# JuliaSmoothOptimizers/CaNNOLeS.jl

Hardware: AMD Instinct MI355X
Metric: Newton systems/sec (fp64), batched n=1e4 NLS; achieved HBM GB/s vs peak (higher is better)
Workload: dtype f64; 1 GPU; cfg3 band constrained NLS n=10000 nequ=10000 ncon=50, 16384 independent problems per GPU, one newton_system! per problem per step; batch_per_gpu=16384, total_problems=16384, ordering=canonical+early, nnzL_stored=145150, nnzL_exact=100180, fronts=1000, all_success=True

## Files before the change

### cannoles.jl_amd/csrc/band.hip

```cpp
#include <hip/hip_runtime.h>

#include "band.h"
#include "kernels.h"

namespace cnl {

namespace {

template <class T>
__device__ __forceinline__ T* as_global(T* p) {
  return (T*)(__attribute__((address_space(1))) T*)p;
}

typedef const __attribute__((address_space(4))) int* cptr;
__device__ __forceinline__ cptr as_const(const int* p) { return (cptr)(const __attribute__((address_space(1))) int*)p; }

constexpr int NPC = BAND_NPIECE;
constexpr int LANE_D = BAND_LANE_DOUBLES;
constexpr int EXCH_OFF = BAND_IN_OFF;
static_assert(48 <= BAND_NPIECE * 8, "exchange area inside the operand pieces");

__device__ __forceinline__ constexpr int sidx(int a, int b) { return a >= b ? a * (a + 1) / 2 + b : b * (b + 1) / 2 + a; }

template <class T>
__device__ __forceinline__ T rrcp(T d) {
  T r;
  if constexpr (sizeof(T) == 8) r = __builtin_amdgcn_rcp(d);
  else r = __builtin_amdgcn_rcpf(d);
  const T e = fma(-d, r, T(1));
  return fma(r, e, r);
}
template <class T>
__device__ __forceinline__ T rdiv(T w, T d, T r) {
  const T q = w * r;
  const T res = fma(-d, q, w);
  return fma(res, r, q);
}


constexpr int NS = BAND_NS;
template <class T>
struct Win {
  T S[NS * (NS + 1) / 2];
  T X[NS];
  T S55;
  T c[NS];
  T c5;
};
__device__ __forceinline__ constexpr int lslot(int PH, int k) { return (PH - BAND_HW + k + NS) % NS; }

#define LDSD(off) (*reinterpret_cast<const T*>(myb + (off)))
#define LDSW(off) (*reinterpret_cast<T*>(myb + (off)))

struct Rec { int v[BAND_SW]; };
struct RowRec { int v[BAND_RW]; };
__device__ __forceinline__ void load_rec(Rec& R, const char* recb, int o) {
  const int4* q = reinterpret_cast<const int4*>(recb + 4 * o);
#pragma unroll
  for (int k = 0; k < BAND_SW / 4; k++) { const int4 t = q[k]; R.v[4 * k] = t.x; R.v[4 * k + 1] = t.y; R.v[4 * k + 2] = t.z; R.v[4 * k + 3] = t.w; }
}
__device__ __forceinline__ void load_row(RowRec& R, const char* recb, int o) {
  const int4* q = reinterpret_cast<const int4*>(recb + 4 * o);
#pragma unroll
  for (int k = 0; k < BAND_RW / 4; k++) { const int4 t = q[k]; R.v[4 * k] = t.x; R.v[4 * k + 1] = t.y; R.v[4 * k + 2] = t.z; R.v[4 * k + 3] = t.w; }
}

template <class T>
struct FOps { T eo[15]; T rj[BAND_NB]; T rdr, rrr; };
template <class T>
__device__ __forceinline__ void fload(FOps<T>& P, const Rec& st, const RowRec& row0, const int fl, char* myb) {
#pragma unroll
  for (int q = 0; q < 15; q++) P.eo[q] = LDSD(st.v[BS_DG0 + q]);
  static_assert(BS_RX == BS_DG0 + 14, "the fifteen operands of an entering variable are consecutive words of the step block");
  P.rdr = T(1); P.rrr = T(0);
#pragma unroll
  for (int k = 0; k < BAND_NB; k++) P.rj[k] = T(0);
  if ((fl >> 8) & 255) {
#pragma unroll
    for (int k = 0; k < BAND_NB; k++) P.rj[k] = LDSD(row0.v[BR_J0 + k]);
    P.rdr = LDSD(row0.v[BR_DI]);
    P.rrr = LDSD(row0.v[BR_RR]);
  }
}

__device__ __forceinline__ long long band_il_offset(int e, int stride) { return stride ? (long long)(e >> 3) * stride + (e & 7) : (long long)e; }

template <int PH, class T>
__device__ __forceinline__ void fstep(Win<T>& W, const FOps<T>& OP, const Rec& st, const int fl, const char* recb, const int o, char* myb,
                                      const T* __restrict__ gvals, const T* __restrict__ grhs, cptr borders, long long pv, long long pr,
                                      bool has_rhs, T rho, bool ovr, T tol, int& npos, int& nzer, const int vstride = 0, const int rstride = 0) {
  constexpr int es = PH, ps = lslot(PH, 0);
  const int nrows = (fl >> 8) & 255;
  const T (&eo)[15] = OP.eo;
  const T (&rj)[BAND_NB] = OP.rj;
  const T rdr = OP.rdr, rrr = OP.rrr;
  {
    const T dg = (eo[0] + eo[1]) + eo[2];
    T rv = eo[BS_RHO - BS_DG0];
    if (!(fl & (1 << 16))) rv = ovr ? rho : rv;
    W.S[sidx(es, es)] = dg + rv;
#pragma unroll
    for (int k = 1; k <= BAND_HW; k++) W.S[sidx(es, lslot(PH, BAND_HW - k))] = eo[BS_OD - BS_DG0 + 2 * (k - 1)] + eo[BS_OD - BS_DG0 + 2 * (k - 1) + 1];
    W.X[es] = eo[BS_BC0 - BS_DG0] + eo[BS_BC1 - BS_DG0];
    W.c[es] = eo[BS_RX - BS_DG0];
  }
  for (int i = 0; i < nrows; i++) {
    T J[BAND_NB], dr, rr;
    if (i == 0) {
#pragma unroll
      for (int k = 0; k < BAND_NB; k++) J[k] = rj[k];
      dr = rdr; rr = rrr;
    } else {
      RowRec rb;
      load_row(rb, recb, o + BAND_SW + BAND_RW * i);
#pragma unroll
      for (int k = 0; k < BAND_NB; k++) J[k] = LDSD(rb.v[BR_J0 + k]);
      dr = LDSD(rb.v[BR_DI]);
      rr = LDSD(rb.v[BR_RR]);
    }
    npos += dr > tol;
    nzer += fabs(dr) <= tol;
    const T r = rrcp(dr);
    const T w = rdiv(T(-1), dr, r);
    const T tr = rr * w;
#pragma unroll
    for (int ka = 0; ka < BAND_NB; ka++) {
      const T ta = J[ka] * w;
#pragma unroll
      for (int kb = 0; kb <= ka; kb++) W.S[sidx(lslot(PH, ka), lslot(PH, kb))] = fma(ta, J[kb], W.S[sidx(lslot(PH, ka), lslot(PH, kb))]);
      W.c[lslot(PH, ka)] = fma(tr, J[ka], W.c[lslot(PH, ka)]);
    }
  }
  if (fl & BF_PIVOT_B) {
    cptr bt = borders + BAND_BW * __builtin_amdgcn_readfirstlane(st.v[BS_BORDER]);
    W.S55 += gvals[pv + band_il_offset(bt[BB_DSRC], vstride)];
    W.c5 += has_rhs ? grhs[pr + band_il_offset(bt[BB_RHS], rstride)] : T(0);
    const T d = W.S55;
    npos += d > tol;
    nzer += fabs(d) <= tol;
    const T r = rrcp(d);
    T l[BAND_NB], w[BAND_NB];
#pragma unroll
    for (int k = 0; k < BAND_NB; k++) { w[k] = W.X[lslot(PH, k)]; l[k] = rdiv(w[k], d, r); }
    const T z = rdiv(W.c5, d, r);
#pragma unroll
    for (int ka = 0; ka < BAND_NB; ka++) {
#pragma unroll
      for (int kb = 0; kb <= ka; kb++) W.S[sidx(lslot(PH, ka), lslot(PH, kb))] = fma(w[ka], -l[kb], W.S[sidx(lslot(PH, ka), lslot(PH, kb))]);
      W.c[lslot(PH, ka)] = fma(w[ka], -z, W.c[lslot(PH, ka)]);
    }
    T* lo = reinterpret_cast<T*>(myb + st.v[BS_LB]);
#pragma unroll
    for (int k = 0; k < BAND_NB; k++) lo[k] = l[k];
    lo[BAND_NB] = z;
#pragma unroll
    for (int k = 0; k < BAND_NB; k++) W.X[lslot(PH, k)] = T(0);
    W.S55 = T(0); W.c5 = T(0);
  }
  if (fl & BF_PIVOT_X) {
    const T d = W.S[sidx(ps, ps)];
    npos += d > tol;
    nzer += fabs(d) <= tol;
    const T r = rrcp(d);
    T l[BAND_NB], w[BAND_NB];
#pragma unroll
    for (int k = 1; k < BAND_NB; k++) { w[k] = W.S[sidx(lslot(PH, k), ps)]; l[k] = rdiv(w[k], d, r); }
    const T w5 = W.X[ps], l5 = rdiv(w5, d, r), z = rdiv(W.c[ps], d, r);
#pragma unroll
    for (int ka = 1; ka < BAND_NB; ka++) {
#pragma unroll
      for (int kb = 1; kb <= ka; kb++) W.S[sidx(lslot(PH, ka), lslot(PH, kb))] = fma(w[ka], -l[kb], W.S[sidx(lslot(PH, ka), lslot(PH, kb))]);
      W.X[lslot(PH, ka)] = fma(w5, -l[ka], W.X[lslot(PH, ka)]);
      W.c[lslot(PH, ka)] = fma(w[ka], -z, W.c[lslot(PH, ka)]);
    }
    W.S55 = fma(w5, -l5, W.S55);
    W.c5 = fma(w5, -z, W.c5);
    T* lo = reinterpret_cast<T*>(myb + st.v[BS_LX]);
#pragma unroll
    for (int k = 1; k < BAND_NB; k++) lo[k - 1] = l[k];
    lo[4] = l5;
    lo[5] = z;
  }
}

template <class T>
struct BOps { T lx[BAND_LREC], lb[BAND_LREC], rj[BAND_NB]; T rdr, rrr; };
template <class T>
__device__ __forceinline__ void bload(BOps<T>& P, const Rec& st, const RowRec& row0, const int fl, char* myb) {
#pragma unroll
  for (int q = 0; q < BAND_LREC; q++) { P.lx[q] = T(0); P.lb[q] = T(0); }
#pragma unroll
  for (int k = 0; k < BAND_NB; k++) P.rj[k] = T(0);
  P.rdr = T(1); P.rrr = T(0);
  if (fl & BF_PIVOT_X) {
    const T* lo = reinterpret_cast<const T*>(myb + st.v[BS_LX]);
#pragma unroll
    for (int q = 0; q < BAND_LREC; q++) P.lx[q] = lo[q];
  }
  if (fl & BF_PIVOT_B) {
    const T* lo = reinterpret_cast<const T*>(myb + st.v[BS_LB]);
#pragma unroll
    for (int q = 0; q < BAND_LREC; q++) P.lb[q] = lo[q];
  }
  if ((fl >> 8) & 255) {
#pragma unroll
    for (int k = 0; k < BAND_NB; k++) P.rj[k] = LDSD(row0.v[BR_J0 + k]);
    P.rdr = LDSD(row0.v[BR_DI]);
    P.rrr = LDSD(row0.v[BR_RR]);
  }
}
template <int PH, class T>
__device__ __forceinline__ void bstep(T (&xs)[NS + 1], const BOps<T>& OP, const Rec& st, const RowRec& row0, const int fl, const char* recb,
                                      const int o, char* myb, cptr borders, T* __restrict__ gd, long long pd, bool okme) {
  constexpr int ps = lslot(PH, 0);
  const int nrows = (fl >> 8) & 255;
  const T (&lx)[BAND_LREC] = OP.lx;
  const T (&lb)[BAND_LREC] = OP.lb;
  const T (&rj)[BAND_NB] = OP.rj;
  const T rdr = OP.rdr, rrr = OP.rrr;
  if (fl & BF_PIVOT_X) {
    T x = lx[5];
#pragma unroll
    for (int k = 1; k < BAND_NB; k++) x = fma(-lx[k - 1], xs[lslot(PH, k)], x);
    x = fma(-lx[4], xs[NS], x);
    xs[ps] = x;
    LDSW(st.v[BS_DX]) = -x;
  }
  if (fl & BF_PIVOT_B) {
    T x = lb[BAND_NB];
#pragma unroll
    for (int k = 0; k < BAND_NB; k++) x = fma(-lb[k], xs[lslot(PH, k)], x);
    xs[NS] = x;
    if (okme) gd[pd + borders[BAND_BW * __builtin_amdgcn_readfirstlane(st.v[BS_BORDER]) + BB_DOUT]] = -x;
  }
  for (int i = 0; i < nrows; i++) {
    T J[BAND_NB], dr, rr;
    int dro;
    if (i == 0) {
#pragma unroll
      for (int k = 0; k < BAND_NB; k++) J[k] = rj[k];
      dr = rdr; rr = rrr; dro = row0.v[BR_DR];
    } else {
      RowRec rb;
      load_row(rb, recb, o + BAND_SW + BAND_RW * i);
#pragma unroll
      for (int k = 0; k < BAND_NB; k++) J[k] = LDSD(rb.v[BR_J0 + k]);
      dr = LDSD(rb.v[BR_DI]); rr = LDSD(rb.v[BR_RR]); dro = rb.v[BR_DR];
    }
    T acc = -rr;
#pragma unroll
    for (int k = 0; k < BAND_NB; k++) acc = fma(J[k], xs[lslot(PH, k)], acc);
    LDSW(dro) = rdiv(acc, dr, rrcp(dr));
  }
  if (fl & BF_ENTER_B) xs[NS] = T(0);
}

}

template <class T, int NL>
__global__ void __launch_bounds__(128, (NL <= 8 ? 2 : 1)) band_newton_kernel(const BandDev P, const LaunchArgs Ain) {
  constexpr int NI = NL / 8;
  constexpr int ES = (int)sizeof(T), LS = ES == 8 ? 3 : 2;
  static_assert(ES == 8 || ES == 4, "double or float");
  extern __shared__ double lds[];
  const int mode = Ain.mode, batch = Ain.batch;
  T* const gvals = as_global(reinterpret_cast<T*>(Ain.vals));
  const T* const grhs = as_global(reinterpret_cast<const T*>(Ain.rhs));
  T* const gd = as_global(reinterpret_cast<T*>(Ain.d));
  T* const gL = as_global(reinterpret_cast<T*>(Ain.L));
  const int lane = threadIdx.x & 63;
  const int part = __builtin_amdgcn_readfirstlane((int)(threadIdx.x >> 6));
  const int lq = lane >> 3, le = lane & 7;
  const int prob0 = blockIdx.x * NL;
  const bool has_rhs = mode != MODE_FACTOR && grhs != nullptr;
  T* const ldsT = reinterpret_cast<T*>(lds);
  char* wblk = reinterpret_cast<char*>(ldsT + (size_t)part * NL * LANE_D);
  char* recb = reinterpret_cast<char*>(ldsT + (size_t)P.nparts * NL * LANE_D) + (size_t)part * BAND_REC_MAX * 4;
  double* ctrl = reinterpret_cast<double*>(reinterpret_cast<char*>(ldsT + (size_t)P.nparts * NL * LANE_D) + (size_t)P.nparts * BAND_REC_MAX * 4);
  const int* fops_g = as_global(P.fops[part]);
  const int* bops_g = as_global(P.bops[part]);
  cptr epochs = as_const(P.epochs[part]);
  cptr borders = as_const(P.borders[part]);
  const int nepochs = P.nepochs[part];
  const int nnz = P.nnz, N = P.N;
  const long long lsize = P.lsize;
  constexpr int G8 = BAND_IL_GROUP * 8;
  static_assert(BAND_IL_GROUP % NL == 0, "a workgroup's problems lie in one group of the interleaved layout");
  const bool vil = (Ain.layout & 1) != 0, ril = (Ain.layout & 2) != 0;
  const int vstride = vil ? G8 : 0, rstride = ril ? G8 : 0;
  const long long ilg = prob0 / BAND_IL_GROUP;
  const int ilp = (prob0 % BAND_IL_GROUP) * 8;
  const T* vbase = gvals + (vil ? ilg * band_il_blocks(nnz) * G8 + ilp : (long long)prob0 * nnz);
  const T* rbase = !has_rhs ? gvals : grhs + (ril ? ilg * band_il_blocks(N) * G8 + ilp : (long long)prob0 * N);
  constexpr bool LINT = NL >= 32;
  T* lbase_g = gL + (long long)prob0 * lsize + (LINT ? 0 : P.loff[part]);
  const int loff8 = LINT ? (int)P.loff[part] : 0;
  T* dbase = gd ? gd + (long long)prob0 * N : nullptr;
  unsigned movp[NI], ldsb[NI];
  bool movok[NI];
#pragma unroll
  for (int i = 0; i < NI; i++) {
    int pl = i * 8 + lq;
    movok[i] = prob0 + pl < batch;
    if (!movok[i]) pl = batch - 1 - prob0;
    movp[i] = (unsigned)pl;
    ldsb[i] = ((unsigned)(i * 8 + lq) * (unsigned)LANE_D + (unsigned)le) << LS;
  }
  const bool clane = lane < NL;
  const int cprob = prob0 + (clane ? lane : 0);
  const bool valid = clane && cprob < batch;
  const int cpl = valid ? cprob - prob0 : batch - 1 - prob0;
  char* myb = wblk + (size_t)(clane ? lane : 0) * LANE_D * ES;
  const long long pv = vil ? ilg * band_il_blocks(nnz) * G8 + ilp + cpl * 8 : (long long)(prob0 + cpl) * nnz;
  const long long pr = ril ? ilg * band_il_blocks(N) * G8 + ilp + cpl * 8 : (long long)(prob0 + cpl) * N;
  for (int t = lane; t < NL; t += 64) *reinterpret_cast<T*>(wblk + ((size_t)t * LANE_D + BAND_ZERO_OFF) * ES) = T(0);

  const T tol = (T)Ain.params[0], kdec = (T)Ain.params[2], kinc = (T)Ain.params[3], klarge = (T)Ain.params[4], rho0 = (T)Ain.params[5],
          rhomax = (T)Ain.params[6], rhomin = (T)Ain.params[7];
  T rho = T(0), wrote = T(0);
  T rho_old = (mode == MODE_NEWTON && valid) ? as_global(reinterpret_cast<T*>(Ain.rho_old))[cprob] : T(0);
  int nfact = 0;
  bool done = !valid, success = false, ovr = false;

  static_assert(NI <= 4, "at most four problem groups per mover lane");
  T stg[NPC][NI];
  int4 rstg0;
  int pcs[NPC];
  static_assert(BAND_REC_MAX <= 256, "record buffer: one dwordx4 per lane");
#define BAND_ISSUE1(K, I) if constexpr (I < NI) stg[K][I] = *reinterpret_cast<const T*>(pb + ((movp[I] * strd + tl) << LS));
#define BAND_COMMIT1(K, I) if constexpr (I < NI) *reinterpret_cast<T*>(wblk + ldsb[I] + (BAND_IN_OFF + 8 * K) * ES) = stg[K][I];
#define BAND_ISSUE(K)                                                                                                         \
  if (pcs[K] >= 0) {                                                                                      \
    const int pc = pcs[K];                                                                                                    \
    const int arr = pc >> 28;                                                                                                 \
    const int el_ = (pc & ((1 << 28) - 1)) + (arr == 2 ? loff8 : 0);                                                          \
                    \
    const bool il_ = arr == 0 ? vil : arr == 1 ? ril : LINT;                                              \
    const int ilw_ = arr == 2 ? NL * 8 : BAND_IL_GROUP * 8;     \
    const int m_ = il_ ? (el_ & 7) : 0;                                                                                       \
    const unsigned gap_ = il_ ? (unsigned)(ilw_ - 8) : 0u;                                                                    \
    const char* pb = (arr == 0 ? reinterpret_cast<const char*>(vbase) : arr == 1 ? reinterpret_cast<const char*>(rbase)       \
                                                                                 : reinterpret_cast<const char*>(lbase_g)) +   \
                     ((il_ ? (long long)(el_ >> 3) * ilw_ : (long long)el_) << LS);                                           \
    const unsigned strd = il_ ? 8u : arr == 0 ? (unsigned)nnz : arr == 1 ? (unsigned)N : (unsigned)lsize;                     \
    const unsigned t_ = (unsigned)m_ + (unsigned)le;                                                                          \
    const unsigned tl = t_ + (t_ >> 3) * gap_;                                                                                \
    BAND_ISSUE1(K, 0) BAND_ISSUE1(K, 1) BAND_ISSUE1(K, 2) BAND_ISSUE1(K, 3)                                                   \
  }
#define BAND_COMMIT(K) { BAND_COMMIT1(K, 0) BAND_COMMIT1(K, 1) BAND_COMMIT1(K, 2) BAND_COMMIT1(K, 3) }
#define BAND_ISSUE_DESC(EP, OFS) { cptr E_ = (EP) + (OFS); _Pragma("unroll") for (int k_ = 0; k_ < NPC; k_++) pcs[k_] = E_[k_]; }
#define BAND_ISSUE_REC(OPS, OPOFF) { rstg0 = (reinterpret_cast<const int4*>((OPS) + (OPOFF)) + lane)[0]; }
#define BAND_ISSUE_ALL(EP, OFS, OPS, OPOFF)                                                                                   \
  {                                                                                                                           \
    BAND_ISSUE_DESC(EP, OFS)                                                                                                  \
    BAND_ISSUE(0) BAND_ISSUE(1) BAND_ISSUE(2) BAND_ISSUE(3) BAND_ISSUE(4) BAND_ISSUE(5) BAND_ISSUE(6) BAND_ISSUE(7)           \
    BAND_ISSUE(8) BAND_ISSUE(9) BAND_ISSUE(10) BAND_ISSUE(11) BAND_ISSUE(12) BAND_ISSUE(13) BAND_ISSUE(14)                    \
    BAND_ISSUE_REC(OPS, OPOFF)                                                                                                \
  }
#define BAND_COMMIT_ALL()                                                                                                     \
  {                                                                                                                           \
    BAND_COMMIT(0) BAND_COMMIT(1) BAND_COMMIT(2) BAND_COMMIT(3) BAND_COMMIT(4) BAND_COMMIT(5) BAND_COMMIT(6) BAND_COMMIT(7)   \
    BAND_COMMIT(8) BAND_COMMIT(9) BAND_COMMIT(10) BAND_COMMIT(11) BAND_COMMIT(12) BAND_COMMIT(13) BAND_COMMIT(14)             \
    reinterpret_cast<int4*>(recb)[lane] = rstg0;                                                                              \
  }
  static_assert(NPC == 15, "fifteen operand pieces");

  Win<T> W;
  int npos = 0, nzer = 0;
  T lj[6], zj[4];
  for (int q = 0; q < 6; q++) lj[q] = T(0);
  for (int q = 0; q < 4; q++) zj[q] = T(0);
  while (true) {
#pragma unroll
    for (int q = 0; q < NS * (NS + 1) / 2; q++) W.S[q] = T(0);
#pragma unroll
    for (int q = 0; q < NS; q++) { W.X[q] = T(0); W.c[q] = T(0); }
    W.S55 = T(0); W.c5 = T(0);
    npos = 0; nzer = 0;
    BAND_ISSUE_ALL(epochs, BE_FP, fops_g, 0)
    for (int e = 0; e < nepochs; e++) {
      cptr E = epochs + e * BAND_EW;
      BAND_COMMIT_ALL()
      const bool more_ = e + 1 < nepochs;
      if (more_) BAND_ISSUE_DESC(epochs + (e + 1) * BAND_EW, BE_FP)
      const int nst = E[BE_NSTEP];
      int o = 0;
      Rec stC, stN;
      RowRec rwC, rwN;
      load_rec(stC, recb, 0);
      load_row(rwC, recb, BAND_SW);
#define BAND_FSTEP(PHV)                                                                                                     \
      if (PHV < nst) {                                                                                                      \
        const int fl = __builtin_amdgcn_readfirstlane(stC.v[BS_FLAGS]);                                                     \
        const int onext = o + BAND_SW + BAND_RW * ((fl >> 8) & 255);                                                        \
        if (PHV + 1 < nst) { load_rec(stN, recb, onext); load_row(rwN, recb, onext + BAND_SW); }                            \
        if (clane) {                                                                                                        \
          FOps<T> op_;                                                                                                      \
          fload(op_, stC, rwC, fl, myb);                                                                                    \
          fstep<PHV>(W, op_, stC, fl, recb, o, myb, gvals, grhs, borders, pv, pr, has_rhs, rho, ovr, tol, npos, nzer, vstride, rstride); \
        }                                                                                                                   \
        o = onext; stC = stN; rwC = rwN;                                                                                    \
      }
#define BAND_LFLUSH(LB, LC)                                                                                                 \
      if (mode != MODE_FACTOR) {                                                                                            \
        const int lc_ = (LC);                                                                                               \
        const int lb_ = (LB) + loff8;                                                                                       \
        char* lout = reinterpret_cast<char*>(lbase_g) + ((LINT ? (long long)(lb_ >> 3) * (NL * 8) : (long long)lb_) << LS); \
        const unsigned t_ = (LINT ? (unsigned)(lb_ & 7) : 0u) + (unsigned)le;                                               \
        const unsigned tl = t_ + (LINT ? (t_ >> 3) * (unsigned)(NL * 8 - 8) : 0u);                                          \
        const unsigned lstr_ = LINT ? 8u : (unsigned)lsize;                                                                 \
        constexpr int lcp_ = LINT ? NL * 8 * ES : 8 * ES;                                                                   \
        T lx_[BAND_LOUT_MAX / 8][NI];                                                                                       \
        _Pragma("unroll") for (int cpc = 0; cpc < BAND_LOUT_MAX / 8; cpc++)                                                 \
          _Pragma("unroll") for (int i = 0; i < NI; i++) lx_[cpc][i] = *reinterpret_cast<const T*>(wblk + ldsb[i] + (BAND_LOUT_OFF + 8 * cpc) * ES); \
        _Pragma("unroll") for (int cpc = 0; cpc < BAND_LOUT_MAX / 8; cpc++)                                                 \
          _Pragma("unroll") for (int i = 0; i < NI; i++)                                                                    \
            if (movok[i] && cpc * 8 + le < lc_)                                                                             \
              *reinterpret_cast<T*>(lout + (((movp[i] * lstr_ + tl) << LS) + lcp_ * cpc)) = lx_[cpc][i];                     \
      }
      BAND_FSTEP(0)
      if (more_) { BAND_ISSUE(0) BAND_ISSUE(1) BAND_ISSUE(2) BAND_ISSUE(3) }
      BAND_FSTEP(1)
      if (more_) { BAND_ISSUE(4) BAND_ISSUE(5) BAND_ISSUE(6) BAND_ISSUE(7) }
      BAND_FSTEP(2)
      if (more_) { BAND_ISSUE(8) BAND_ISSUE(9) BAND_ISSUE(10) BAND_ISSUE(11) }
      BAND_FSTEP(3)
      if (more_) { BAND_ISSUE(12) BAND_ISSUE(13) BAND_ISSUE(14) BAND_ISSUE_REC(fops_g, epochs[(e + 1) * BAND_EW + BE_FOFF]) }
      BAND_LFLUSH(E[BE_LBASE], E[BE_LCNT])
      BAND_FSTEP(4) BAND_FSTEP(5) BAND_FSTEP(6) BAND_FSTEP(7)
      static_assert(BAND_EPOCH == 8, "eight step instantiations per epoch");
      if (nst == BAND_EPOCH) {
#pragma unroll
        for (int a = 0; a < NS; a++)
#pragma unroll
          for (int b = 0; b <= a; b++)
            if (b < 4) W.S[sidx(a, b)] = T(0);
#pragma unroll
        for (int a = 0; a < 4; a++) { W.X[a] = T(0); W.c[a] = T(0); }
      }
      BAND_LFLUSH(E[BE_LBASE2], E[BE_LCNT2])
    }
    int tpos = npos, tzer = nzer;
    if (P.nparts == 2) {
      if (clane) {
        T* ex = reinterpret_cast<T*>(myb + EXCH_OFF * ES);
#pragma unroll
        for (int q = 0; q < NS * (NS + 1) / 2; q++) ex[q] = W.S[q];
#pragma unroll
        for (int q = 0; q < NS; q++) ex[36 + q] = W.c[q];
        ex[44] = (T)npos; ex[45] = (T)nzer;
      }
      __syncthreads();
      if (part == 0 && clane) {
        const T* exL = reinterpret_cast<const T*>(myb + EXCH_OFF * ES);
        const T* exR = reinterpret_cast<const T*>(myb + (size_t)NL * LANE_D * ES + EXCH_OFF * ES);
        const int tL = P.m0 % NS, tR = (P.n - 1 - P.m0) % NS;
        T SJ[10], cJ[4];
#pragma unroll
        for (int i = 0; i < 4; i++) {
          const int aL = (tL + i) % NS, aR = (tR - i + NS) % NS;
#pragma unroll
          for (int j = 0; j <= i; j++) {
            const int bL = (tL + j) % NS, bR = (tR - j + NS) % NS;
            const int iL = aL >= bL ? aL * (aL + 1) / 2 + bL : bL * (bL + 1) / 2 + aL;
            const int iR = aR >= bR ? aR * (aR + 1) / 2 + bR : bR * (bR + 1) / 2 + aR;
            SJ[i * (i + 1) / 2 + j] = exL[iL] + exR[iR];
          }
          cJ[i] = exL[36 + aL] + exR[36 + aR];
        }
        tpos += (int)exR[44]; tzer += (int)exR[45];
#pragma unroll
        for (int i = 0; i < 4; i++) {
          const T d = SJ[sidx(i, i)];
          tpos += d > tol;
          tzer += fabs(d) <= tol;
          const T r = rrcp(d);
          zj[i] = rdiv(cJ[i], d, r);
          T w[4];
#pragma unroll
          for (int a = i + 1; a < 4; a++) { w[a] = SJ[sidx(a, i)]; lj[sidx(a - 1, i)] = rdiv(w[a], d, r); }
#pragma unroll
          for (int a = i + 1; a < 4; a++) {
#pragma unroll
            for (int b = i + 1; b <= a; b++) SJ[sidx(a, b)] = fma(w[a], -lj[sidx(b - 1, i)], SJ[sidx(a, b)]);
            cJ[a] = fma(w[a], -zj[i], cJ[a]);
          }
        }
      }
    }
    bool alldone = true;
    if (part == 0) {
      const bool ok = tpos == P.nvar && tzer == 0;
      if (mode == MODE_FACTOR) {
        if (valid) {
          as_global(Ain.success)[cprob] = ok ? 1 : 0;
          if (Ain.npos) as_global(Ain.npos)[cprob] = tpos;
          if (Ain.nzero) as_global(Ain.nzero)[cprob] = tzer;
        }
        done = true;
      } else if (mode == MODE_SOLVE) {
        success = ok;
        done = true;
      } else if (!done) {
        nfact++;
        if (ok) { done = true; success = true; }
        else if (nfact == 1) {
          rho = rho_old == T(0) ? rho0 : fmax(rhomin, kdec * rho_old);
          ovr = true; wrote = rho;
        } else if (rho <= rhomax) {
          rho = rho_old == T(0) ? klarge * rho : kinc * rho;
          if (rho <= rhomax) wrote = rho; else done = true;
        } else done = true;
      }
      alldone = __all(done || !clane);
      if (clane) { ctrl[lane] = rho; ctrl[NL + lane] = (ovr ? 1.0 : 0.0) + (success ? 2.0 : 0.0); }
      if (lane == 0) ctrl[2 * NL] = alldone ? 1.0 : 0.0;
    }
    if (P.nparts == 2) {
      __syncthreads();
      if (part == 1) {
        if (clane) { rho = (T)ctrl[lane]; const int f = (int)ctrl[NL + lane]; ovr = f & 1; success = f & 2; }
        alldone = ctrl[2 * NL] != 0.0;
      }
      __syncthreads();
    }
    if (alldone) break;
  }
  if (mode == MODE_FACTOR) {
    if (mode == MODE_NEWTON && part == 0 && valid) as_global(Ain.success)[cprob] = 1;
    return;
  }
  {
    T xs[NS + 1];
#pragma unroll
    for (int q = 0; q < NS + 1; q++) xs[q] = T(0);
    if (P.nparts == 2) {
      if (part == 0 && clane) {
        T xj[4];
        xj[3] = zj[3];
        xj[2] = fma(-lj[sidx(2, 2)], xj[3], zj[2]);
        xj[1] = fma(-lj[sidx(2, 1)], xj[3], fma(-lj[sidx(1, 1)], xj[2], zj[1]));
        xj[0] = fma(-lj[sidx(2, 0)], xj[3], fma(-lj[sidx(1, 0)], xj[2], fma(-lj[sidx(0, 0)], xj[1], zj[0])));
        T* ex = reinterpret_cast<T*>(myb + EXCH_OFF * ES);
        T* exR = reinterpret_cast<T*>(myb + (size_t)NL * LANE_D * ES + EXCH_OFF * ES);
#pragma unroll
        for (int i = 0; i < 4; i++) {
          ex[i] = xj[i]; exR[i] = xj[i];
          if (valid && success) gd[(long long)cprob * N + P.m0 + i] = -xj[i];
        }
      }
      __syncthreads();
      if (clane) {
        const T* ex = reinterpret_cast<const T*>(myb + EXCH_OFF * ES);
        const int t0 = part == 0 ? P.m0 % NS : (P.n - 1 - P.m0) % NS;
#pragma unroll
        for (int s = 0; s < NS; s++) {
          const int i = part == 0 ? (s - t0 + NS) % NS : (t0 - s + NS) % NS;
          xs[s] = i < 4 ? ex[i] : T(0);
        }
      }
    }
    if (part == 0 && clane) ctrl[NL + lane] = (valid && success) ? 2.0 : 0.0;
    __syncthreads();
    bool movst[NI];
#pragma unroll
    for (int i = 0; i < NI; i++) movst[i] = movok[i] && ctrl[NL + i * 8 + lq] != 0.0;
    const bool okme = valid && ctrl[NL + lane % NL] != 0.0 && clane;
    const long long pd = (long long)(prob0 + cpl) * N;
    BAND_ISSUE_ALL(epochs + (nepochs - 1) * BAND_EW, BE_BP, bops_g, 0)
    for (int e = nepochs - 1; e >= 0; e--) {
      cptr E = epochs + e * BAND_EW;
      BAND_COMMIT_ALL()
      const bool more_ = e > 0;
      if (more_) BAND_ISSUE_DESC(epochs + (e - 1) * BAND_EW, BE_BP)
      const int nst = E[BE_NSTEP];
      int o = 0;
      Rec stC, stN;
      RowRec rwC, rwN;
      load_rec(stC, recb, 0);
      load_row(rwC, recb, BAND_SW);
#define BAND_BSTEP(PHV)                                                                                                     \
      if (PHV < nst) {                                                                                                      \
        const int fl = __builtin_amdgcn_readfirstlane(stC.v[BS_FLAGS]);                                                     \
        const int onext = o + BAND_SW + BAND_RW * ((fl >> 8) & 255);                                                        \
        if (PHV > 0) { load_rec(stN, recb, onext); load_row(rwN, recb, onext + BAND_SW); }                                  \
        if (clane) {                                                                                                        \
          BOps<T> op_;                                                                                                      \
          bload(op_, stC, rwC, fl, myb);                                                                                    \
          bstep<PHV>(xs, op_, stC, rwC, fl, recb, o, myb, borders, gd, pd, okme);                                           \
        }                                                                                                                   \
        o = onext; stC = stN; rwC = rwN;                                                                                    \
      }
      BAND_BSTEP(7)
      if (more_) { BAND_ISSUE(0) BAND_ISSUE(1) BAND_ISSUE(2) BAND_ISSUE(3) }
      BAND_BSTEP(6)
      if (more_) { BAND_ISSUE(4) BAND_ISSUE(5) BAND_ISSUE(6) BAND_ISSUE(7) }
      BAND_BSTEP(5)
      if (more_) { BAND_ISSUE(8) BAND_ISSUE(9) BAND_ISSUE(10) BAND_ISSUE(11) }
      BAND_BSTEP(4)
      if (more_) { BAND_ISSUE(12) BAND_ISSUE(13) BAND_ISSUE(14) BAND_ISSUE_REC(bops_g, epochs[(e - 1) * BAND_EW + BE_BOFF]) }
      BAND_BSTEP(3) BAND_BSTEP(2) BAND_BSTEP(1) BAND_BSTEP(0)
      const int xlo = E[BE_DXLO], xc = E[BE_DXCNT], rlo = E[BE_DRLO], rc = E[BE_DRCNT];
      char* dxo = reinterpret_cast<char*>(dbase) + ((long long)xlo << LS);
      char* dro = reinterpret_cast<char*>(dbase) + ((long long)rlo << LS);
      {
        T dx_[NI], dr_[BAND_DR_MAX / 8][NI];
#pragma unroll
        for (int i = 0; i < NI; i++) dx_[i] = *reinterpret_cast<const T*>(wblk + ldsb[i] + BAND_DX_OFF * ES);
#pragma unroll
        for (int cpc = 0; cpc < BAND_DR_MAX / 8; cpc++)
#pragma unroll
          for (int i = 0; i < NI; i++) dr_[cpc][i] = *reinterpret_cast<const T*>(wblk + ldsb[i] + (BAND_DR_OFF + 8 * cpc) * ES);
#pragma unroll
        for (int i = 0; i < NI; i++)
          if (movst[i] && le < xc) *reinterpret_cast<T*>(dxo + ((movp[i] * (unsigned)N + (unsigned)le) << LS)) = dx_[i];
#pragma unroll
        for (int cpc = 0; cpc < BAND_DR_MAX / 8; cpc++)
#pragma unroll
          for (int i = 0; i < NI; i++)
            if (movst[i] && cpc * 8 + le < rc) *reinterpret_cast<T*>(dro + (((movp[i] * (unsigned)N + (unsigned)le) << LS) + 8 * ES * cpc)) = dr_[cpc][i];
      }
    }
  }
  if (part == 0 && mode == MODE_NEWTON) {
    if (nfact > 1 && rho <= rhomax) rho_old = rho;
    if (valid) {
      as_global(reinterpret_cast<T*>(Ain.rho))[cprob] = rho;
      as_global(reinterpret_cast<T*>(Ain.rho_old))[cprob] = rho_old;
      as_global(Ain.nfact)[cprob] = nfact;
      as_global(Ain.success)[cprob] = success ? 1 : 0;
    }
    for (int q = 0; q < NL; q++) {
      const int nf = __builtin_amdgcn_readlane(nfact, q);
      const int vq = __builtin_amdgcn_readlane((int)valid, q);
      if (nf > 1 && vq) {
        T wq;
        if constexpr (ES == 8) wq = __hiloint2double(__builtin_amdgcn_readlane(__double2hiint(wrote), q), __builtin_amdgcn_readlane(__double2loint(wrote), q));
        else wq = __int_as_float(__builtin_amdgcn_readlane(__float_as_int(wrote), q));
        if (vil) {
          T* vg = gvals + ilg * band_il_blocks(nnz) * G8 + ilp + q * 8;
          for (int i = lane; i < P.nvar; i += 64) vg[band_il_offset(nnz - P.nvar + i, vstride)] = wq;
        } else {
          T* vt = gvals + (long long)(prob0 + q) * nnz + (nnz - P.nvar);
          for (int i = lane; i < P.nvar; i += 64) vt[i] = wq;
        }
      }
    }
  }
}

size_t band_lds_bytes(int nparts, int nl, int esz) {
  return (size_t)nparts * nl * LANE_D * esz + (2 * (size_t)nl + 8) * sizeof(double) + (size_t)nparts * BAND_REC_MAX * 4;
}

template <class T>
static hipError_t launch_band_t(const BandDev& P, int nl, const LaunchArgs& a, hipStream_t stream) {
  const size_t ldsb = band_lds_bytes(P.nparts, nl, (int)sizeof(T));
  const int grid = (a.batch + nl - 1) / nl;
  auto go = [&](auto kern) {
    hipError_t e = hipFuncSetAttribute(reinterpret_cast<const void*>(kern), hipFuncAttributeMaxDynamicSharedMemorySize, lds_attr_cap((int)ldsb));
    if (e != hipSuccess) return e;
    hipLaunchKernelGGL(kern, dim3(grid), dim3(64 * P.nparts), ldsb, stream, P, a);
    return hipGetLastError();
  };
  if (nl == 32) return go(band_newton_kernel<T, 32>);
  if (nl == 16) return go(band_newton_kernel<T, 16>);
  if (nl == 8) return go(band_newton_kernel<T, 8>);
  return hipErrorInvalidConfiguration;
}

hipError_t launch_band(const BandDev& P, int nl, const LaunchArgs& a, hipStream_t stream) { return launch_band_t<double>(P, nl, a, stream); }
hipError_t launch_band_f32(const BandDev& P, int nl, const LaunchArgs& a, hipStream_t stream) { return launch_band_t<float>(P, nl, a, stream); }

}
```

Measured before the change: 1.456 million systems/s.

## Defer per-epoch global stores into next epoch to overlap with compute

The L-output flush in the factor sweep and the dx/dr stores in the backward sweep are now read from LDS into registers at the end of each epoch and written to global memory after the first step of the next epoch, so the stores overlap with computation instead of stalling at epoch boundaries. In the factor sweep this is gated by a constexpr condition (fp32 or NL>=16), so it may not apply to every configuration, while the backward-sweep deferral always applies. The two-part junction back-solve for xj is also moved earlier, next to where lj/zj are computed, which removes those long-lived register arrays. The deferred values cost extra registers held across a whole epoch, which can lower occupancy.

```diff
diff --git a/cannoles.jl_amd/csrc/band.hip b/cannoles.jl_amd/csrc/band.hip
--- a/cannoles.jl_amd/csrc/band.hip
+++ b/cannoles.jl_amd/csrc/band.hip
@@ -367,9 +367,6 @@
 
   Win<T> W;
   int npos = 0, nzer = 0;
-  T lj[6], zj[4];
-  for (int q = 0; q < 6; q++) lj[q] = T(0);
-  for (int q = 0; q < 4; q++) zj[q] = T(0);
   while (true) {
 #pragma unroll
     for (int q = 0; q < NS * (NS + 1) / 2; q++) W.S[q] = T(0);
@@ -378,6 +375,9 @@
     W.S55 = T(0); W.c5 = T(0);
     npos = 0; nzer = 0;
     BAND_ISSUE_ALL(epochs, BE_FP, fops_g, 0)
+    constexpr bool LHOLD = ES == 4 || NL >= 16;
+    T lh_[BAND_LOUT_MAX / 8][NI];
+    int lhb = 0, lhc = 0;
     for (int e = 0; e < nepochs; e++) {
       cptr E = epochs + e * BAND_EW;
       BAND_COMMIT_ALL()
@@ -401,8 +401,11 @@
         }                                                                                                                   \
         o = onext; stC = stN; rwC = rwN;                                                                                    \
       }
-#define BAND_LFLUSH(LB, LC)                                                                                                 \
-      if (mode != MODE_FACTOR) {                                                                                            \
+#define BAND_LREAD(H)                                                                                                       \
+      _Pragma("unroll") for (int cpc = 0; cpc < BAND_LOUT_MAX / 8; cpc++)                                                   \
+        _Pragma("unroll") for (int i = 0; i < NI; i++) (H)[cpc][i] = *reinterpret_cast<const T*>(wblk + ldsb[i] + (BAND_LOUT_OFF + 8 * cpc) * ES);
+#define BAND_LSTORE(H, LB, LC)                                                                                              \
+      {                                                                                                                     \
         const int lc_ = (LC);                                                                                               \
         const int lb_ = (LB) + loff8;                                                                                       \
         char* lout = reinterpret_cast<char*>(lbase_g) + ((LINT ? (long long)(lb_ >> 3) * (NL * 8) : (long long)lb_) << LS); \
@@ -410,15 +413,19 @@
         const unsigned tl = t_ + (LINT ? (t_ >> 3) * (unsigned)(NL * 8 - 8) : 0u);                                          \
         const unsigned lstr_ = LINT ? 8u : (unsigned)lsize;                                                                 \
         constexpr int lcp_ = LINT ? NL * 8 * ES : 8 * ES;                                                                   \
-        T lx_[BAND_LOUT_MAX / 8][NI];                                                                                       \
-        _Pragma("unroll") for (int cpc = 0; cpc < BAND_LOUT_MAX / 8; cpc++)                                                 \
-          _Pragma("unroll") for (int i = 0; i < NI; i++) lx_[cpc][i] = *reinterpret_cast<const T*>(wblk + ldsb[i] + (BAND_LOUT_OFF + 8 * cpc) * ES); \
         _Pragma("unroll") for (int cpc = 0; cpc < BAND_LOUT_MAX / 8; cpc++)                                                 \
           _Pragma("unroll") for (int i = 0; i < NI; i++)                                                                    \
             if (movok[i] && cpc * 8 + le < lc_)                                                                             \
-              *reinterpret_cast<T*>(lout + (((movp[i] * lstr_ + tl) << LS) + lcp_ * cpc)) = lx_[cpc][i];                     \
+              *reinterpret_cast<T*>(lout + (((movp[i] * lstr_ + tl) << LS) + lcp_ * cpc)) = (H)[cpc][i];                     \
+      }
+#define BAND_LFLUSH(LB, LC)                                                                                                 \
+      if (mode != MODE_FACTOR) {                                                                                            \
+        T lx_[BAND_LOUT_MAX / 8][NI];                                                                                       \
+        BAND_LREAD(lx_)                                                                                                     \
+        BAND_LSTORE(lx_, LB, LC)                                                                                            \
       }
       BAND_FSTEP(0)
+      if (LHOLD && mode != MODE_FACTOR && e > 0) BAND_LSTORE(lh_, lhb, lhc)
       if (more_) { BAND_ISSUE(0) BAND_ISSUE(1) BAND_ISSUE(2) BAND_ISSUE(3) }
       BAND_FSTEP(1)
       if (more_) { BAND_ISSUE(4) BAND_ISSUE(5) BAND_ISSUE(6) BAND_ISSUE(7) }
@@ -438,8 +445,12 @@
 #pragma unroll
         for (int a = 0; a < 4; a++) { W.X[a] = T(0); W.c[a] = T(0); }
       }
-      BAND_LFLUSH(E[BE_LBASE2], E[BE_LCNT2])
-    }
+      if constexpr (LHOLD) {
+        if (mode != MODE_FACTOR) { BAND_LREAD(lh_) }
+        lhb = E[BE_LBASE2]; lhc = E[BE_LCNT2];
+      } else BAND_LFLUSH(E[BE_LBASE2], E[BE_LCNT2])
+    }
+    if (LHOLD && mode != MODE_FACTOR && nepochs > 0) BAND_LSTORE(lh_, lhb, lhc)
     int tpos = npos, tzer = nzer;
     if (P.nparts == 2) {
       if (clane) {
@@ -469,6 +480,7 @@
           cJ[i] = exL[36 + aL] + exR[36 + aR];
         }
         tpos += (int)exR[44]; tzer += (int)exR[45];
+        T lj[6], zj[4];
 #pragma unroll
         for (int i = 0; i < 4; i++) {
           const T d = SJ[sidx(i, i)];
@@ -486,6 +498,15 @@
             cJ[a] = fma(w[a], -zj[i], cJ[a]);
           }
         }
+        T xj[4];
+        xj[3] = zj[3];
+        xj[2] = fma(-lj[sidx(2, 2)], xj[3], zj[2]);
+        xj[1] = fma(-lj[sidx(2, 1)], xj[3], fma(-lj[sidx(1, 1)], xj[2], zj[1]));
+        xj[0] = fma(-lj[sidx(2, 0)], xj[3], fma(-lj[sidx(1, 0)], xj[2], fma(-lj[sidx(0, 0)], xj[1], zj[0])));
+        T* xL = reinterpret_cast<T*>(myb + EXCH_OFF * ES);
+        T* xR = reinterpret_cast<T*>(myb + (size_t)NL * LANE_D * ES + EXCH_OFF * ES);
+#pragma unroll
+        for (int i = 0; i < 4; i++) { xL[i] = xj[i]; xR[i] = xj[i]; }
       }
     }
     bool alldone = true;
@@ -535,19 +556,10 @@
 #pragma unroll
     for (int q = 0; q < NS + 1; q++) xs[q] = T(0);
     if (P.nparts == 2) {
-      if (part == 0 && clane) {
-        T xj[4];
-        xj[3] = zj[3];
-        xj[2] = fma(-lj[sidx(2, 2)], xj[3], zj[2]);
-        xj[1] = fma(-lj[sidx(2, 1)], xj[3], fma(-lj[sidx(1, 1)], xj[2], zj[1]));
-        xj[0] = fma(-lj[sidx(2, 0)], xj[3], fma(-lj[sidx(1, 0)], xj[2], fma(-lj[sidx(0, 0)], xj[1], zj[0])));
-        T* ex = reinterpret_cast<T*>(myb + EXCH_OFF * ES);
-        T* exR = reinterpret_cast<T*>(myb + (size_t)NL * LANE_D * ES + EXCH_OFF * ES);
-#pragma unroll
-        for (int i = 0; i < 4; i++) {
-          ex[i] = xj[i]; exR[i] = xj[i];
-          if (valid && success) gd[(long long)cprob * N + P.m0 + i] = -xj[i];
-        }
+      if (part == 0 && clane && valid && success) {
+        const T* ex = reinterpret_cast<const T*>(myb + EXCH_OFF * ES);
+#pragma unroll
+        for (int i = 0; i < 4; i++) gd[(long long)cprob * N + P.m0 + i] = -ex[i];
       }
       __syncthreads();
       if (clane) {
@@ -568,6 +580,19 @@
     const bool okme = valid && ctrl[NL + lane % NL] != 0.0 && clane;
     const long long pd = (long long)(prob0 + cpl) * N;
     BAND_ISSUE_ALL(epochs + (nepochs - 1) * BAND_EW, BE_BP, bops_g, 0)
+    T dh_[NI], rh_[BAND_DR_MAX / 8][NI];
+    int hxlo = 0, hxc = 0, hrlo = 0, hrc = 0;
+#define BAND_DSTORE()                                                                                                       \
+    {                                                                                                                       \
+      char* dxo = reinterpret_cast<char*>(dbase) + ((long long)hxlo << LS);                                                 \
+      char* dro = reinterpret_cast<char*>(dbase) + ((long long)hrlo << LS);                                                 \
+      _Pragma("unroll") for (int i = 0; i < NI; i++)                                                                        \
+        if (movst[i] && le < hxc) *reinterpret_cast<T*>(dxo + ((movp[i] * (unsigned)N + (unsigned)le) << LS)) = dh_[i];    \
+      _Pragma("unroll") for (int cpc = 0; cpc < BAND_DR_MAX / 8; cpc++)                                                     \
+        _Pragma("unroll") for (int i = 0; i < NI; i++)                                                                      \
+          if (movst[i] && cpc * 8 + le < hrc)                                                                               \
+            *reinterpret_cast<T*>(dro + (((movp[i] * (unsigned)N + (unsigned)le) << LS) + 8 * ES * cpc)) = rh_[cpc][i];     \
+    }
     for (int e = nepochs - 1; e >= 0; e--) {
       cptr E = epochs + e * BAND_EW;
       BAND_COMMIT_ALL()
@@ -592,6 +617,7 @@
         o = onext; stC = stN; rwC = rwN;                                                                                    \
       }
       BAND_BSTEP(7)
+      if (e < nepochs - 1) BAND_DSTORE()
       if (more_) { BAND_ISSUE(0) BAND_ISSUE(1) BAND_ISSUE(2) BAND_ISSUE(3) }
       BAND_BSTEP(6)
       if (more_) { BAND_ISSUE(4) BAND_ISSUE(5) BAND_ISSUE(6) BAND_ISSUE(7) }
@@ -600,27 +626,15 @@
       BAND_BSTEP(4)
       if (more_) { BAND_ISSUE(12) BAND_ISSUE(13) BAND_ISSUE(14) BAND_ISSUE_REC(bops_g, epochs[(e - 1) * BAND_EW + BE_BOFF]) }
       BAND_BSTEP(3) BAND_BSTEP(2) BAND_BSTEP(1) BAND_BSTEP(0)
-      const int xlo = E[BE_DXLO], xc = E[BE_DXCNT], rlo = E[BE_DRLO], rc = E[BE_DRCNT];
-      char* dxo = reinterpret_cast<char*>(dbase) + ((long long)xlo << LS);
-      char* dro = reinterpret_cast<char*>(dbase) + ((long long)rlo << LS);
-      {
-        T dx_[NI], dr_[BAND_DR_MAX / 8][NI];
-#pragma unroll
-        for (int i = 0; i < NI; i++) dx_[i] = *reinterpret_cast<const T*>(wblk + ldsb[i] + BAND_DX_OFF * ES);
-#pragma unroll
-        for (int cpc = 0; cpc < BAND_DR_MAX / 8; cpc++)
-#pragma unroll
-          for (int i = 0; i < NI; i++) dr_[cpc][i] = *reinterpret_cast<const T*>(wblk + ldsb[i] + (BAND_DR_OFF + 8 * cpc) * ES);
-#pragma unroll
-        for (int i = 0; i < NI; i++)
-          if (movst[i] && le < xc) *reinterpret_cast<T*>(dxo + ((movp[i] * (unsigned)N + (unsigned)le) << LS)) = dx_[i];
-#pragma unroll
-        for (int cpc = 0; cpc < BAND_DR_MAX / 8; cpc++)
-#pragma unroll
-          for (int i = 0; i < NI; i++)
-            if (movst[i] && cpc * 8 + le < rc) *reinterpret_cast<T*>(dro + (((movp[i] * (unsigned)N + (unsigned)le) << LS) + 8 * ES * cpc)) = dr_[cpc][i];
-      }
-    }
+#pragma unroll
+      for (int i = 0; i < NI; i++) dh_[i] = *reinterpret_cast<const T*>(wblk + ldsb[i] + BAND_DX_OFF * ES);
+#pragma unroll
+      for (int cpc = 0; cpc < BAND_DR_MAX / 8; cpc++)
+#pragma unroll
+        for (int i = 0; i < NI; i++) rh_[cpc][i] = *reinterpret_cast<const T*>(wblk + ldsb[i] + (BAND_DR_OFF + 8 * cpc) * ES);
+      hxlo = E[BE_DXLO]; hxc = E[BE_DXCNT]; hrlo = E[BE_DRLO]; hrc = E[BE_DRCNT];
+    }
+    if (nepochs > 0) BAND_DSTORE()
   }
   if (part == 0 && mode == MODE_NEWTON) {
     if (nfact > 1 && rho <= rhomax) rho_old = rho;
```

Result: faster. 1.473 million systems/s (median of 6 runs) (+1.2%).
